# zetanumbers/myraytracer

Measured on AMD Instinct MI355X. Metric: Msamples/s (pixels x spp / s), random-spheres, higher is better.
Workload: dtype f32

## Files before the change

myraytracer_amd/csrc/kernels.hip:

```cpp

#include <hip/hip_runtime.h>
#include "mrt_internal.h"
#include "mrt_device.h"
#include "sweep.h"
#include "blend.h"

#include <type_traits>

namespace mrt {
namespace {

__device__ __forceinline__ float sphere_quadratic(float cx, float cy, float cz, float neg_r2, V3 o, V3 d, float a, float& b, float& c) {
    const float ocx = o.x - cx, ocy = o.y - cy, ocz = o.z - cz;
    b = __builtin_fmaf(ocz, d.z, __builtin_fmaf(ocy, d.y, ocx * d.x));
    c = __builtin_fmaf(ocz, ocz, __builtin_fmaf(ocy, ocy, __builtin_fmaf(ocx, ocx, neg_r2)));
    return __builtin_fmaf(b, b, -(a * c));
}
__device__ __forceinline__ void literal_test(const SphereRec s, uint32_t idx, V3 o, V3 d, float a,
                                             float& t_sup, int32_t& best) {
    float b, c;
    const float disc = sphere_quadratic(s.cx, s.cy, s.cz, s.neg_r2, o, d, a, b, c);
    if (!(disc < 0.0f)) {
        float d_sqrt = __builtin_sqrtf(disc);
        const float t_min = 0.001f;
// ... 159 lines not shown
    const SphereRec* nodes = SMALL ? reinterpret_cast<const SphereRec*>(lds_raw) : P.nodes;
    const uint32_t* __restrict__ member_index = P.member_index;
    const SphQuadPtr sph_quads = (SphQuadPtr)(uintptr_t)P.clusters;
    const float pixel_side = 2.0f / (float)H;

    auto locate = [&](KArgPtr C, uint32_t q, uint32_t& px, uint32_t& py, uint32_t& texel, uint32_t& layer) -> bool {
        uint32_t tile = q >> 6;
        const uint32_t l = q & 63u;
        layer = 0u;
        if (!PILOT && C->queue_layers > 1u) { layer = tile / C->n_tiles; tile -= layer * C->n_tiles; }
        const uint32_t tile_x = tile % C->tiles_x, band = tile / C->tiles_x;
        const uint32_t Wc = C->locals.shape[0], Hc = C->locals.shape[1];
        px = tile_x * kTileW + (l & 7u);
        py = (band * C->shard_world + C->shard_rank) * kBandRows + (l >> 3);
        texel = (band * kBandRows + (l >> 3)) * Wc + px;
        return px < Wc && py < Hc;
    };

    uint32_t head = 0, tail = 0, avail = 0;
    bool queue_empty = false;

    bool has_task = false, task_done = false;
    uint32_t s_done = 0, pix_trips = 0, texel = 0;
    float base_x = 0.0f, base_y = 0.0f;
    Rng rng; rng.draws = 0; rng.s0 = rng.s1 = rng.s2 = rng.s3 = 0;
    uint32_t blk = 0;
    V3 color = v3(0.0f, 0.0f, 0.0f);
    V3 o = v3(0.0f, 0.0f, 0.0f), d = v3(0.0f, 0.0f, -1.0f), att = v3(1.0f, 1.0f, 1.0f);
    uint32_t depth_left = 0, trips = 0;
    unsigned long long started = 0, bounces = 0;
    unsigned long long mtests = 0;
    unsigned long long prim_slots = 0;

#ifdef MRT_STAMPS
    uint64_t phase_[7] = {0, 0, 0, 0, 0, 0, 0};
    uint64_t rounds_a_ = 0, rounds_b_ = 0, items_a_ = 0, items_b_ = 0;
    uint64_t last_ = __builtin_amdgcn_s_memtime();
    const uint64_t wave_t0_ = __builtin_amdgcn_s_memrealtime();
#endif

    for (;;) {
        const bool live = has_task && !task_done;
        auto new_sample_head = [&](V3& nd, V3& p) -> bool {
            if (CTR) {
                const KArgPtr Cs = cold_args();
                const uint4 sd = reinterpret_cast<const uint4*>(Cs->seeds)[texel];
                const uint32_t k4 = 4u * ((blk >> 7) * kCtrBlock + s_done);
                rng.s0 = fmix32((sd.x ^ Cs->locals.rng_shuffle[0]) + 0x9E3779B9u * (k4 + 1u));
                rng.s1 = fmix32((sd.y ^ Cs->locals.rng_shuffle[1]) + 0x9E3779B9u * (k4 + 2u));
                rng.s2 = fmix32((sd.z ^ Cs->locals.rng_shuffle[2]) + 0x9E3779B9u * (k4 + 3u));
                rng.s3 = fmix32((sd.w ^ Cs->locals.rng_shuffle[3]) + 0x9E3779B9u * (k4 + 4u));
                if ((rng.s0 | rng.s1 | rng.s2 | rng.s3) == 0u) {
                    rng.s0 = 0x9E3779B9u; rng.s1 = 0x7F4A7C15u; rng.s2 = 0xBF58476Du; rng.s3 = 0x1CE4E5B9u;
                }
            }
            float u = rng_f32(rng); float v = rng_f32(rng);
            float vx = base_x + u * pixel_side;
            float vy = base_y + v * pixel_side;
            const KArgPtr C = cold_args();
            att = v3(1.0f, 1.0f, 1.0f);
            depth_left = C->locals.ray_depth;
            if (C->cam.mode == 0) {
                o = v3(0.0f, 0.0f, 0.0f);
                nd = v3(vx, vy, -1.0f);
                return false;
            }
            p = v3((vx * C->cam.su[0] + vy * C->cam.sv[0]) - C->cam.fw[0],
                   (vx * C->cam.su[1] + vy * C->cam.sv[1]) - C->cam.fw[1],
                   (vx * C->cam.su[2] + vy * C->cam.sv[2]) - C->cam.fw[2]);
            o = v3(C->cam.origin[0], C->cam.origin[1], C->cam.origin[2]);
            nd = p;
            return C->cam.defocus != 0;
        };
        auto new_sample_lens = [&](V3& nd, V3 p, float lx, float ly) {
            const KArgPtr C = cold_args();
            const V3 off = v3(lx * C->cam.ru[0] + ly * C->cam.rv[0],
                              lx * C->cam.ru[1] + ly * C->cam.rv[1],
                              lx * C->cam.ru[2] + ly * C->cam.rv[2]);
            o = o + off;
            nd = p - off;
        };
        trips++;

        const bool trace = live && depth_left != 0u;
        if (trace) pix_trips++;
        if (!PILOT) bounces += (uint32_t)__popcll(__builtin_amdgcn_ballot_w64(trace));
        float t_sup = 1.0e4f;
        int32_t best = -1;
        if (__any(trace)) {
            const float a = dot3(d, d);
            constexpr bool CAM = SMALL && !DBG && !LISTS;
            bool cam_on = false;
            uint4 cam_entry = make_uint4(0xFFFFFFFFu, 0xFFFFFFFFu, 0xFFFFFFFFu, 0xFFFFFFFFu);
            if constexpr (CAM) {
                const KArgPtr C = cold_args();
                const uint32_t* const cam_masks = C->cam_masks;
                cam_on = cam_masks != nullptr;
                if (cam_on && trace && depth_left == C->locals.ray_depth) cam_entry = reinterpret_cast<const uint4*>(cam_masks)[texel >> 3];
            }
            auto cam_allow = [&](const uint32_t w) -> uint32_t {
                uint32_t allow = 0xFFFFFFFFu;
                if constexpr (CAM) { if (cam_on) allow = masks[w * 64u]; }
                return allow;
            };
            V3 o_rel = MFMA ? v3(o.x - P.mfma_origin[0], o.y - P.mfma_origin[1], o.z - P.mfma_origin[2]) : o;
            const float stretch = MFMA ? P.mfma_scale[0] : kBoundStretch;
            V3 ds = v3(d.x * stretch, d.y * stretch, d.z * stretch);
            if (MFMA && P.mfma_scaled != 0u) {
                o_rel = v3(o_rel.x * P.mfma_axis[0], o_rel.y * P.mfma_axis[1], o_rel.z * P.mfma_axis[2]);
                const V3 dd = v3(d.x * P.mfma_axis[0], d.y * P.mfma_axis[1], d.z * P.mfma_axis[2]);
                const float unit = __builtin_amdgcn_rsqf(dot3(dd, dd)) * stretch;
                ds = v3(dd.x * unit, dd.y * unit, dd.z * unit);
            }
            const float o_rel2 = MFMA ? dot3(o_rel, o_rel) : 0.0f;
            const bool weird = !(a > 0.99999f && a < 1.00001f) || (MFMA && !(o_rel2 <= P.mfma_scale[3]));
            const bool usable = trace && !weird;
            unsigned long long key0 = kNoHitKey;
            {
                const KArgPtr C = cold_args();
                const uint32_t n_direct = C->n_direct;
                const Divisor by_a = divisor_of(a);
                for (uint32_t j = 0; j < n_direct; j++) {
                    const float cx = C->direct[j].cx, cy = C->direct[j].cy, cz = C->direct[j].cz, nr2 = C->direct[j].neg_r2;
                    const uint32_t sidx = C->direct_index[j];
                    bool hq;
                    const unsigned long long key = sphere_root_key(cx, cy, cz, nr2, sidx, o, d, a, by_a, usable, hq);
                    key0 = key < key0 ? key : key0;
                    if (DBG && hq) atomicOr(P.dbg_cand + (size_t)texel * P.dbg_words + (sidx >> 5), 1u << (sidx & 31u));
                }
                if (!PILOT) mtests += (unsigned long long)n_direct * (uint32_t)__popcll(__builtin_amdgcn_ballot_w64(usable));
            }
            rays[2u * lane + 0u] = make_float4(o.x, o.y, o.z, d.x);
            rays[2u * lane + 1u] = make_float4(d.y, d.z, __uint_as_float((uint32_t)key0), __uint_as_float((uint32_t)(key0 >> 32)));
            lds_order();
            uint32_t bits = 0;
            MfmaRay mr;
            if (MFMA) mr = mfma_ray_operands(o_rel, ds, o_rel2, P.mfma_scale[1], P.mfma_scale[2], P.mfma_neg_k2_pair);
            if (CAM && cam_on) {
                masks[0] = cam_entry.x;
                if (n_padded > 32u) masks[64] = cam_entry.y;
                if (n_padded > 64u) masks[128] = cam_entry.z;
                if (n_padded > 96u) masks[192] = cam_entry.w;
                lds_order();
            }
            for (uint32_t blk = 0; blk < n_padded; blk += kBlockChunks * kChunk) {
                const uint32_t blk_end = (blk + kBlockChunks * kChunk < n_padded) ? blk + kBlockChunks * kChunk : n_padded;
                uint32_t nz = 0;
                uint32_t rem = 0;
                if (MFMA) {
                    uint32_t w = 0;
                    for (uint32_t i = blk; i < blk_end; i += 2u * kChunk, w++) {
                        const uint32_t allow = cam_allow(w);
                        uint32_t m = mfma_sweep_tile(reinterpret_cast<const u32x4*>(P.top_mfma)[(size_t)(i / 32u) * 64u + lane], mr);
                        if constexpr (CAM) m &= allow;
                        masks[w * 64u] = m;
                        nz |= (m < 1u ? m : 1u) << w;
                        rem += (uint32_t)__builtin_popcount(m);
                    }
                } else {
                Sph8 ga, gb;
                smem_load8(ga, sph_quads, blk);
                asm volatile("" : "=s"(gb.lo), "=s"(gb.hi));
                uint32_t c = 0;
                for (uint32_t i = blk; i < blk_end; i += kChunk, c++) {
                    const uint32_t allow = cam_allow(c >> 1);
                    smem_wait_then_load8(ga, gb, sph_quads, i + 8u, bits);  test8(ga, o, ds, bits);
                    const uint32_t nxt = (i + kChunk < n_padded) ? i + kChunk : 0u;
                    smem_wait_then_load8(gb, ga, sph_quads, nxt, bits);
                    test8(gb, o, ds, bits);
                    if (c & 1u) {
                        uint32_t m = ~bits;
                        if constexpr (CAM) m &= allow;
                        masks[(c >> 1) * 64u] = m;
                        nz |= (m < 1u ? m : 1u) << (c >> 1);
                        rem += (uint32_t)__builtin_popcount(m);
                    }
                }
                asm volatile("s_waitcnt lgkmcnt(0)" : "+s"(ga.lo), "+s"(ga.hi), "+s"(gb.lo), "+s"(gb.hi));
                }
                MRT_STAMP(1);
                if (!usable) { nz = 0; rem = 0; }
                lds_order();

                uint32_t wm = 0, ebase = 0;
                auto fetch_ray = [&](const uint32_t owner, V3& ro, V3& rd) {
                    const float4 r0 = rays[2u * owner];
                    const float2 r1 = *reinterpret_cast<const float2*>(rays + 2u * owner + 1u);
                    ro = v3(r0.x, r0.y, r0.z), rd = v3(r0.w, r1.x, r1.y);
                };
                auto root_round = [&](const entry_t* const src, uint32_t& n) {
                    const uint32_t take = n < 64u ? n : 64u, start = n - take;
                    const bool act = lane < take;
                    const uint32_t it = src[act ? start + lane : 0u];
                    const uint32_t owner = it >> kIdBits, node = it & ((1u << kIdBits) - 1u);
                    V3 ro, rd;
                    fetch_ray(owner, ro, rd);
                    const float ra = dot3(rd, rd);
                    const SphereRec sm = nodes[node];
                    const uint32_t sidx = SMALL ? (uint32_t)index_lds[node] : member_index[node];
                    float bq, cq;
                    const float disc = sphere_quadratic(sm.cx, sm.cy, sm.cz, sm.neg_r2, ro, rd, ra, bq, cq);
                    const float d_sqrt = sqrt_unscaled(disc);
                    const float t_min = 0.001f;
                    const Divisor by_a = divisor_of(ra);
                    const float t_near = div_unscaled(-bq - d_sqrt, by_a);
                    const float t_far = div_unscaled(-bq + d_sqrt, by_a);
                    const bool ok_near = !(t_near < t_min) && t_near < 1.0e4f;
                    const bool ok_far = !(t_far < t_min) && t_far < 1.0e4f;
                    const float t = ok_near ? t_near : t_far;
                    const unsigned long long key = (act && (ok_near || ok_far)) ? (((unsigned long long)__float_as_uint(t) << 32) | sidx) : kNoHitKey;
                    atomicMin(best_slots + 4u * owner, key);
                    if (DBG) {
                        const uint32_t owner_ray = (uint32_t)__builtin_amdgcn_ds_bpermute((int)(owner << 2), (int)texel);
                        if (act) atomicOr(P.dbg_cand + (size_t)owner_ray * P.dbg_words + (sidx >> 5), 1u << (sidx & 31u));
                    }
                    n = start;
#ifdef MRT_STAMPS
                    rounds_b_++; items_b_ += take;
#endif
                    lds_order();
                    MRT_WALK_STAMP(3);
                };
                auto members_round = [&](const SphereRec* const ch, const V3 ro, const V3 rd, const float ra, const bool on,
                                         const uint32_t e0, entry_t* const dst) -> uint32_t {
                    const SphereRec sr[4] = {ch[0], ch[1], ch[2], ch[3]};
                    bool h[4];
                    unsigned long long hm[4];
#pragma unroll
                    for (int q = 0; q < 4; q++) {
                        float bq, cq;
                        const float disc = sphere_quadratic(sr[q].cx, sr[q].cy, sr[q].cz, sr[q].neg_r2, ro, rd, ra, bq, cq);
                        h[q] = (int32_t)((__float_as_uint(bq) | __float_as_uint(cq)) & ~__float_as_uint(disc)) < 0;
                        hm[q] = __builtin_amdgcn_ballot_w64(h[q]);
                    }
                    const unsigned long long on_mask = __builtin_amdgcn_ballot_w64(on);
                    const unsigned long long m0 = hm[0] & on_mask, m1 = hm[1] & on_mask, m2 = hm[2] & on_mask, m3 = hm[3] & on_mask;
                    const unsigned long long any = m0 | m1 | m2 | m3;
                    const unsigned long long twice = (m0 & m1) | ((m0 | m1) & m2) | ((m0 | m1 | m2) & m3);
                    if (twice == 0ull) {
                        const uint32_t q = h[1] ? 1u : h[2] ? 2u : h[3] ? 3u : 0u;
                        if ((h[0] || h[1] || h[2] || h[3]) && on) dst[rank_in(any)] = (entry_t)(e0 + q);
                        return (uint32_t)__popcll(any);
                    }
                    uint32_t pushed = 0;
#pragma unroll
                    for (int q = 0; q < 4; q++) {
                        const unsigned long long mk = hm[q] & on_mask;
                        if (h[q] && on) dst[pushed + rank_in(mk)] = (entry_t)(e0 + (uint32_t)q);
                        pushed += (uint32_t)__popcll(mk);
                    }
                    return pushed;
                };
                if constexpr (SMALL) {
                    uint32_t qn0 = 0;
                    entry_t* const q0 = queues;
                    uint32_t* const starts = reinterpret_cast<uint32_t*>(queues + kQueueCap);
                    const uint32_t* const masks0 = masks - lane;
                    const uint32_t words = (blk_end - blk) / (2u * kChunk);
                    const bool own = rem != 0u;
                    const unsigned long long own_mask = __builtin_amdgcn_ballot_w64(own);
                    if (own_mask != 0ull) {
                        const uint32_t w0 = own ? 31u - (uint32_t)__builtin_clz(nz) : 0u;
                        const uint32_t m0 = masks[w0 * 64u];
                        const uint32_t node = blk + w0 * (2u * kChunk) + (own ? 31u - (uint32_t)__builtin_ctz(m0) : 0u);
                        qn0 += members_round(nodes + 4u * node, o, d, a, own, (lane << kIdBits) | (4u * node), q0 + qn0);
                        if (!PILOT) mtests += kClusterK * (uint32_t)__popcll(own_mask);
#ifdef MRT_STAMPS
                        rounds_a_++; items_a_ += (uint32_t)__popcll(own_mask);
#endif
                        lds_order();
                        MRT_WALK_STAMP(2);
                        while (qn0 >= 64u) root_round(q0, qn0);
                    }
                    const uint32_t rest = rem - (own ? 1u : 0u);
                    const uint32_t incl = wave_incl_scan(rest);
                    const uint32_t total_rem = (uint32_t)__builtin_amdgcn_readlane((int)incl, 63);
                    const uint32_t start_entry = rest != 0u ? ((incl - rest) << 6) | lane : 0xFFFFFFFFu;
                    uint32_t carry = 0u;
                    auto pick_word = [&](auto NW, const uint32_t owner, const uint32_t r, uint32_t& sel, uint32_t& r_in) -> uint32_t {
                        constexpr int n = decltype(NW)::value;
                        const uint32_t* const mo = masks0 + (int32_t)(words - (uint32_t)n) * 64 + owner;
                        uint32_t cnt = 0u, above = 0u, below = 0u;
                        bool found = false;
                        sel = 0u;
#pragma unroll
                        for (int i = n - 1; i >= 0; i--) {
                            const uint32_t m = mo[i * 64];
                            sel = found ? sel : m;
                            above = found ? above : cnt;
                            cnt += (uint32_t)__builtin_popcount(m);
                            found = r < cnt;
                            below += found ? 0u : 1u;
                        }
                        r_in = r - above;
                        return blk + (words - 1u - below) * (2u * kChunk);
                    };
                    for (uint32_t base = 0; base < total_rem; base += kItemWindow) {
#pragma unroll
                        for (uint32_t i = 0; i < kItemWindow; i += 64u) starts[i + lane] = 0u;
                        lds_order();
                        if ((start_entry >> 6) - base < kItemWindow) starts[(start_entry >> 6) - base] = start_entry;
                        lds_order();
                        const uint32_t window_end = total_rem - base < kItemWindow ? total_rem : base + kItemWindow;
                        for (uint32_t g0 = base; g0 < window_end; g0 += 64u) {
                            const uint32_t take = total_rem - g0 < 64u ? total_rem - g0 : 64u;
                            const bool act = lane < take;
                            uint32_t e = starts[g0 - base + lane];
                            e = wave_incl_max(e < carry ? carry : e);
                            carry = (uint32_t)__builtin_amdgcn_readlane((int)e, 63);
                            const uint32_t owner = e & 63u;
                            const uint32_t r = g0 + (act ? lane : take - 1u) - (e >> 6) + 1u;
                            uint32_t sel, r_in;
                            const uint32_t first = words <= 4u ? pick_word(IC<4>{}, owner, r, sel, r_in) : pick_word(IC<8>{}, owner, r, sel, r_in);
                            for (uint32_t trip = 0; trip < 31u && __any(r_in != 0u); trip++) {
                                if (r_in != 0u) { sel &= sel - 1u; r_in--; }
                            }
                            const uint32_t node = first + 31u - (uint32_t)__builtin_ctz(sel);
                            V3 ro, rd;
                            fetch_ray(owner, ro, rd);
                            MRT_WALK_STAMP(6);
                            qn0 += members_round(nodes + 4u * node, ro, rd, dot3(rd, rd), act, (owner << kIdBits) | (4u * node), q0 + qn0);
                            if (!PILOT) mtests += kClusterK * take;
#ifdef MRT_STAMPS
                            rounds_a_++; items_a_ += take;
#endif
                            lds_order();
                            MRT_WALK_STAMP(2);
                            while (qn0 >= 64u) root_round(q0, qn0);
                        }
                    }
                    while (qn0 != 0u) root_round(q0, qn0);
                } else {
                    constexpr uint32_t kIndexMask = (1u << 26) - 1u;
                    uint32_t sn = 0, cn = 0, rn = 0;
                    uint32_t* const clusterq = queues;
                    uint32_t* const rootq = queues + kQueueCap;
                    uint32_t* const stack = queues + 2u * kQueueCap;
                    typedef float f32x4 __attribute__((ext_vector_type(4)));
                    typedef float f32x2 __attribute__((ext_vector_type(2)));
                    typedef const f32x4 __attribute__((address_space(3)))* LdsBoxPtr;
                    typedef const f32x4 __attribute__((address_space(1)))* GlobalBoxPtr;
                    typedef const f32x2 __attribute__((address_space(3)))* LdsBox2Ptr;
                    typedef const f32x2 __attribute__((address_space(1)))* GlobalBox2Ptr;
                    auto f4 = [](const f32x4 v) { return make_float4(v.x, v.y, v.z, v.w); };
                    const LdsBoxPtr bxs_lds = (LdsBoxPtr)lds_raw;
                    const GlobalBoxPtr bxs_g = (GlobalBoxPtr)P.boxes;
                    const LdsBox2Ptr bx2_lds = (LdsBox2Ptr)lds_raw;
                    const GlobalBox2Ptr bx2_g = (GlobalBox2Ptr)P.boxes;
                    const float box_kc = P.box_kc;
                    const uint32_t box_lds = P.box_lds_count;
                    const bool top_in_lds = box_lds >= n_padded;
                    const uint32_t cluster_parent_first = P.box_cluster_parent_first;
                    for (;;) {
                        int k = rn >= 64u ? 0 : cn >= 64u ? 1 : sn >= 64u ? 2 : -1;
                        if (k < 0) {
                            if (__any((nz | wm) != 0u)) {
                                uint32_t qn = levels == 1u ? cn : sn;
                                uint32_t* const dst = levels == 1u ? clusterq : stack;
                                const uint32_t owner_bits = lane << 26;
                                auto next_candidate = [&]() -> uint32_t {
                                    uint32_t code = 0u;
                                    if ((nz | wm) != 0u) {
                                        if (wm == 0u) refill_mask_word(nz, wm, masks, ebase, 0u, blk);
                                        code = 0x80000000u | take_mask_bit(wm, ebase);
                                    }
                                    return code;
                                };
                                auto fetch_box = [&](const uint32_t code, V3& bc, V3& be) {
                                    const uint32_t g = code & 0x7FFFFFFFu;
                                    f32x2 w0, w1, w2;
                                    if (top_in_lds) { w0 = bx2_lds[3u * g]; w1 = bx2_lds[3u * g + 1u]; w2 = bx2_lds[3u * g + 2u]; }
                                    else { w0 = bx2_g[3u * (size_t)g]; w1 = bx2_g[3u * (size_t)g + 1u]; w2 = bx2_g[3u * (size_t)g + 2u]; }
                                    bc = v3(w0.x, w0.y, w1.x);
                                    be = v3(w1.y, w2.x, w2.y);
                                };
                                auto test_push = [&](const uint32_t code, const V3 bc, const V3 be) {
                                    const bool keep = (int32_t)(box_separated_bits<QUAD>(bc, be, box_kc, o, d) | ~code) >= 0;
                                    const unsigned long long km = __builtin_amdgcn_ballot_w64(keep);
                                    if (keep) dst[qn + rank_in(km)] = owner_bits | (code & 0x7FFFFFFFu);
                                    qn += (uint32_t)__popcll(km);
                                };
                                auto some_left = [&](const uint32_t code) -> bool { return __builtin_amdgcn_ballot_w64((int32_t)code < 0) != 0ull; };
                                uint32_t ca = next_candidate(), cb, left;
                                V3 a0, a1, b0, b1;
                                fetch_box(ca, a0, a1);
                                for (;;) {
                                    cb = next_candidate();
                                    fetch_box(cb, b0, b1);
                                    test_push(ca, a0, a1);
                                    if (!(some_left(cb) && qn < 128u)) { left = cb; break; }
                                    ca = next_candidate();
                                    fetch_box(ca, a0, a1);
                                    test_push(cb, b0, b1);
                                    if (!(some_left(ca) && qn < 128u)) { left = ca; break; }
                                }
                                if ((int32_t)left < 0) wm |= 0x80000000u >> ((left & 0x7FFFFFFFu) - ebase);
                                if (levels == 1u) cn = qn; else sn = qn;
                                lds_order();
                                MRT_WALK_STAMP(6);
                                continue;
                            }
                            k = sn != 0u ? 2 : cn != 0u ? 1 : rn != 0u ? 0 : -1;
                            if (k < 0) break;
                        }
                        if (k == 0) { root_round(rootq, rn); continue; }
                        const uint32_t n = k == 1 ? cn : sn;
                        uint32_t take = n < 64u ? n : 64u;
                        if (k == 2) {
                            const uint32_t fit = gen_cap > sn ? (gen_cap - sn) / 3u : 0u;
                            take = take <= fit ? take : (fit ? fit : 1u);
                        }
                        const uint32_t start = n - take;
                        const bool act = lane < take;
                        const uint32_t it = (k == 1 ? clusterq : stack)[act ? start + lane : 0u];
                        const uint32_t owner = it >> 26, g = act ? it & kIndexMask : 0u;
                        V3 ro, rd;
                        fetch_ray(owner, ro, rd);
                        if (k == 1) {
                            const uint32_t m4 = act ? 4u * (g - P.box_cluster_first) : 0u;
                            rn += members_round(nodes + m4, ro, rd, dot3(rd, rd), act, (owner << 26) | m4, rootq + rn);
                            cn = start;
                            if (!PILOT) mtests += kClusterK * take;
                        } else {
                            const uint32_t c0 = 4u * g + n_padded;
                            float4 b[6];
                            if (__builtin_amdgcn_ballot_w64(act && c0 + 4u > box_lds) == 0ull) {
                                const LdsBoxPtr bx = bxs_lds + 6u * (c0 >> 2);
#pragma unroll
                                for (int q = 0; q < 6; q++) b[q] = f4(bx[q]);
                            } else {
                                const GlobalBoxPtr bx = bxs_g + 6u * (size_t)(c0 >> 2);
#pragma unroll
                                for (int q = 0; q < 6; q++) b[q] = f4(bx[q]);
                            }
                            const V3 bc[4] = {v3(b[0].x, b[0].y, b[0].z), v3(b[1].z, b[1].w, b[2].x), v3(b[3].x, b[3].y, b[3].z), v3(b[4].z, b[4].w, b[5].x)};
                            const V3 be[4] = {v3(b[0].w, b[1].x, b[1].y), v3(b[2].y, b[2].z, b[2].w), v3(b[3].w, b[4].x, b[4].y), v3(b[5].y, b[5].z, b[5].w)};
                            bool h[4];
                            unsigned long long hm[4];
                            const unsigned long long act_mask = __builtin_amdgcn_ballot_w64(act);
#pragma unroll
                            for (int q = 0; q < 4; q++) {
                                h[q] = box_may_touch<QUAD>(bc[q], be[q], box_kc, ro, rd);
                                hm[q] = __builtin_amdgcn_ballot_w64(h[q]) & act_mask;
                            }
                            sn = start;
                            const bool to_c = g >= cluster_parent_first;
                            const unsigned long long m_c = __builtin_amdgcn_ballot_w64(to_c) & act_mask, m_s = act_mask & ~m_c;
                            const uint32_t e0 = (owner << 26) | c0;
                            auto push4 = [&](uint32_t* const dst, const unsigned long long who, const bool mine) -> uint32_t {
                                uint32_t pushed = 0;
#pragma unroll
                                for (int q = 0; q < 4; q++) {
                                    const unsigned long long mk = hm[q] & who;
                                    if (h[q] && mine) dst[pushed + rank_in(mk)] = e0 + (uint32_t)q;
                                    pushed += (uint32_t)__popcll(mk);
                                }
                                return pushed;
                            };
                            if (m_s != 0ull) sn += push4(stack + sn, m_s, act && !to_c);
                            if (m_c != 0ull) cn += push4(clusterq + cn, m_c, act && to_c);
                        }
#ifdef MRT_STAMPS
                        rounds_a_++; items_a_ += take;
#endif
                        lds_order();
                        MRT_WALK_STAMP(2);
                    }
                }
            }
            if (trace) {
                if (weird) {
                    for (uint32_t idx = 0; idx < P.n_spheres; idx++)
                        literal_test(spheres[idx], idx, o, d, a, t_sup, best);
                } else {
                    const unsigned long long key = best_slots[4u * lane];
                    t_sup = __uint_as_float((uint32_t)(key >> 32));
                    best = (int32_t)(uint32_t)key;
                }
            }
        }
        MRT_WALK_STAMP(3);
        if (DBG && live) {
            P.dbg_hit[2u * texel] = best;
            P.dbg_hit[2u * texel + 1u] = (int32_t)__float_as_uint(t_sup);
            task_done = true;
        }

        bool start_sample = false;
        V3 ndir = d;
        bool hit = !DBG && live && depth_left != 0u && best >= 0;
        if (!DBG && live && !hit) {
            if (depth_left != 0u) {
                float t = 0.5f * d.y + 0.5f;
                color = color + att * v3(mixf(1.0f, 0.5f, t), mixf(1.0f, 0.7f, t), mixf(1.0f, 1.0f, t));
            }
            s_done++;
            if (s_done < (CTR ? (blk & 127u) : spp)) start_sample = true;
            else if (!CTR && !PILOT && blk + 1u < cold_args()->lane_frames) {
                const KArgPtr C = cold_args();
                PixAcc sa; sa.r = color.x; sa.g = color.y; sa.b = color.z; sa.cost = pix_trips;
                reinterpret_cast<PixAcc*>(C->pix_acc)[(size_t)blk * C->pix_stride + texel] = sa;
                blk++;
                const uint4 sd = reinterpret_cast<const uint4*>(C->seeds)[texel];
                rng.s0 = sd.x ^ C->layer_shuffle[blk][0];
                rng.s1 = sd.y ^ C->layer_shuffle[blk][1];
                rng.s2 = sd.z ^ C->layer_shuffle[blk][2];
                rng.s3 = sd.w ^ C->layer_shuffle[blk][3];
                color = v3(0.0f, 0.0f, 0.0f);
                s_done = 0;
                pix_trips = 0;
                start_sample = true;
            } else task_done = true;
        }
        MRT_STAMP(4);

        const bool release = has_task && task_done;
        if (release) {
            if (!DBG) {
                PixAcc sa; sa.r = color.x; sa.g = color.y; sa.b = color.z; sa.cost = pix_trips;
                const KArgPtr C = cold_args();
                reinterpret_cast<PixAcc*>(C->pix_acc)[(size_t)(CTR ? (blk >> 7) : blk) * C->pix_stride + texel] = sa;
            }
            has_task = false;
        }
        const unsigned long long need = __ballot(!has_task);
        if (!queue_empty && avail < (uint32_t)__popcll(need)) {
            const KArgPtr C = cold_args();
            uint32_t t = 0;
            if (lane == 0) t = atomicAdd(C->tile_queue, 1u);
            t = __builtin_amdgcn_readfirstlane(t);
            const uint32_t n_layers = PILOT ? 1u : C->queue_layers;
            if (t >= C->n_tiles * n_layers) {
                queue_empty = true;
            } else {
                const uint32_t lay = PILOT ? 0u : t / C->n_tiles, ti = t - lay * C->n_tiles;
                const uint32_t tile = lay * C->n_tiles + (C->tile_order ? C->tile_order[ti] : ti);
                uint32_t fx, fy, ft, fl;
                const uint32_t fq = (tile << 6) | lane;
                const bool ok = locate(C, fq, fx, fy, ft, fl);
                const unsigned long long m = __ballot(ok);
                if (ok) ring[(tail + rank_in(m)) & (kRingCap - 1u)] = fq;
                const uint32_t nf = (uint32_t)__popcll(m);
                tail += nf;
                avail += nf;
            }
        }
        if (need != 0ull && avail != 0u) {
            const uint32_t rk = rank_in(need);
            const bool take = !has_task && rk < avail;
            if (take) {
                const KArgPtr C = cold_args();
                uint32_t px, py, layer;
                locate(C, ring[(head + rk) & (kRingCap - 1u)], px, py, texel, layer);
                const float Wf = (float)C->locals.shape[0], Hf = (float)C->locals.shape[1];
                base_x = (((float)px + 0.5f) - 0.5f * Wf) * pixel_side;
                base_y = (((float)py + 0.5f) - 0.5f * Hf) * pixel_side;
                const uint4 sd = reinterpret_cast<const uint4*>(C->seeds)[texel];
                const uint32_t li = CTR ? 0u : layer;
                rng.s0 = sd.x ^ C->layer_shuffle[li][0];
                rng.s1 = sd.y ^ C->layer_shuffle[li][1];
                rng.s2 = sd.z ^ C->layer_shuffle[li][2];
                rng.s3 = sd.w ^ C->layer_shuffle[li][3];
                if (!CTR) texel += layer * C->pix_stride;
                color = v3(0.0f, 0.0f, 0.0f);
                s_done = 0;
                pix_trips = 0;
                has_task = true;
                blk = 0u;
                if (CTR) {
                    const uint32_t first = layer * kCtrBlock;
                    const uint32_t cnt = spp > first ? (spp - first < kCtrBlock ? spp - first : kCtrBlock) : 0u;
                    blk = (layer << 7) | cnt;
                }
                task_done = (spp == 0u);
                start_sample = !task_done;
                if (DBG) {
                    const float* const r6 = C->dbg_rays + 6u * (size_t)texel;
                    o = v3(r6[0], r6[1], r6[2]);
                    d = v3(r6[3], r6[4], r6[5]);
                    depth_left = 1u;
                    task_done = false;
                    start_sample = false;
                }
            }
            const uint32_t np = (uint32_t)__popcll(need);
            const uint32_t took = np < avail ? np : avail;
            head += took;
            avail -= took;
        }
        if (!__any(has_task)) {
            if (queue_empty) break;
            continue;
        }
        MRT_STAMP(5);

        if (!DBG) {
            V3 cam_p = v3(0.0f, 0.0f, 0.0f);
            bool need_lens = false;
            bool own_ray = false;
            if constexpr (LISTS) {
                if (__any(start_sample)) {
                    uint4 ent = make_uint4(kCamListOverflow, 0u, 0u, 0u);
                    if (start_sample) {
                        ent = reinterpret_cast<const uint4*>(cold_args()->cam_lists)[texel >> 3];
                        if (new_sample_head(ndir, cam_p)) {
                            float lx, ly;
                            do { lx = rng_pm1(rng); ly = rng_pm1(rng); } while (__builtin_fmaf(ly, ly, lx * lx) > 1.0f);
                            new_sample_lens(ndir, cam_p, lx, ly);
                        }
                        d = unit_direction(ndir);
                        ndir = d;
                        own_ray = true;
                    }
                    const float a = dot3(d, d);
                    const bool prim = start_sample && depth_left != 0u && ent.x != kCamListOverflow && a > 0.99999f && a < 1.00001f;
                    const unsigned long long prim_mask = __builtin_amdgcn_ballot_w64(prim);
                    const KArgPtr C = cold_args();
                    const uint32_t n_direct = C->n_direct;
                    const Divisor by_a = divisor_of(a);
                    unsigned long long key = kNoHitKey;
                    bool hq;
                    for (uint32_t j = 0; j < n_direct; j++) {
                        const unsigned long long kk = sphere_root_key(C->direct[j].cx, C->direct[j].cy, C->direct[j].cz, C->direct[j].neg_r2,
                                                                      C->direct_index[j], o, d, a, by_a, prim, hq);
                        key = kk < key ? kk : key;
                    }
                    if (!PILOT) mtests += (unsigned long long)n_direct * (uint32_t)__popcll(prim_mask);
                    const uint32_t cnt = prim ? ent.x : 0u;
                    uint32_t w0 = ent.y, w1 = ent.z, w2 = ent.w;
                    for (uint32_t k = 0;; k++) {
                        const bool on = k < cnt;
                        const unsigned long long on_mask = __builtin_amdgcn_ballot_w64(on);
                        if (on_mask == 0ull) break;
                        const uint32_t slot = on ? w0 & 1023u : 0u;
                        w0 = __builtin_amdgcn_alignbit(w1, w0, 10u); w1 = __builtin_amdgcn_alignbit(w2, w1, 10u); w2 >>= 10u;
                        const SphereRec sm = nodes[slot];
                        const unsigned long long kk = sphere_root_key(sm.cx, sm.cy, sm.cz, sm.neg_r2, (uint32_t)index_lds[slot], o, d, a, by_a, on, hq);
                        key = kk < key ? kk : key;
                        if (!PILOT) mtests += (uint32_t)__popcll(on_mask);
                    }
                    if (!PILOT) {
                        bounces += (uint32_t)__popcll(prim_mask);
                        prim_slots += (uint32_t)__popcll(prim_mask);
                    }
                    if (prim) {
                        pix_trips++;
                        if ((int32_t)(uint32_t)key >= 0) {
                            t_sup = __uint_as_float((uint32_t)(key >> 32));
                            best = (int32_t)(uint32_t)key;
                            hit = true;
                            own_ray = false;
                        } else {
                            float t = 0.5f * d.y + 0.5f;
                            color = color + att * v3(mixf(1.0f, 0.5f, t), mixf(1.0f, 0.7f, t), mixf(1.0f, 1.0f, t));
                            depth_left = 0u;
                        }
                    }
                }
            } else if (start_sample) need_lens = new_sample_head(ndir, cam_p);
            MRT_TAIL_STAMP(2);
            V3 normal = v3(0.0f, 0.0f, 0.0f), refl = v3(0.0f, 0.0f, 0.0f);
            float fuzz = 0.0f;
            bool is_lambertian = false, is_metal = false;
            if (hit) {
                const KArgPtr C = cold_args();
                const float4 sh0 = reinterpret_cast<const float4*>(C->shade)[2 * best];
                const float4 sh1 = reinterpret_cast<const float4*>(C->shade)[2 * best + 1];
                const int32_t m_ty = C->i32_data[C->world.spheres.material_ty_base_idx + best];
                const V3 center = v3(sh0.x, sh0.y, sh0.z);
                const float radius = sh0.w;
                const V3 at = o + t_sup * d;
                const V3 rel = at - center;
                const float rel_min = __builtin_fminf(__builtin_fminf(__builtin_fabsf(rel.x), __builtin_fabsf(rel.y)), __builtin_fabsf(rel.z));
                if (__builtin_expect(__any(!normal_unscaled_ok(rel_min, radius)), 0)) {
                    normal = rel / radius;
                } else {
                    const Divisor by_r = divisor_of(radius);
                    normal = v3(div_unscaled(rel.x, by_r), div_unscaled(rel.y, by_r), div_unscaled(rel.z, by_r));
                }
                const bool front_face = dot3(normal, d) <= 0.0f;
                if (!front_face) normal = -normal;
                is_lambertian = m_ty == MRT_LAMBERTIAN;
                is_metal = m_ty == MRT_METAL;
                if (is_lambertian || is_metal) {
                    att = att * v3(sh1.x, sh1.y, sh1.z);
                    if (is_metal) { refl = reflect3(d, normal); fuzz = sh1.w; }
                } else if (m_ty == MRT_DIELECTRIC) {
                    const float ior = sh1.w;
                    const float ri = front_face ? sh1.x : ior;
                    const float r0 = front_face ? sh1.y : sh1.z;
                    float cos_t = dot3(-d, normal);
                    cos_t = (cos_t < 1.0f) ? cos_t : 1.0f;
                    const float sin_t = sqrt_unscaled(1.0f - cos_t * cos_t);
                    const bool cannot_refract = (ri * sin_t) > 1.0f;
                    const float x1 = 1.0f - cos_t;
                    const float x2 = x1 * x1; const float x4 = x2 * x2; const float x5 = x4 * x1;
                    const float reflectance = r0 + (1.0f - r0) * x5;
                    const float u = rng_f32(rng);
                    if (cannot_refract || reflectance > u) {
                        ndir = reflect3(d, normal);
                    } else {
                        const V3 perp = v3(ri * (d.x + cos_t * normal.x), ri * (d.y + cos_t * normal.y),
                                           ri * (d.z + cos_t * normal.z));
                        const float k = -sqrt_unscaled(__builtin_fabsf(1.0f - dot3(perp, perp)));
                        ndir = v3(perp.x + k * normal.x, perp.y + k * normal.y, perp.z + k * normal.z);
                    }
                } else {
                    depth_left = 1u;
                    ndir = d;
                }
                o = at;
            }
            MRT_TAIL_STAMP(3);
            const bool need_ball = is_lambertian || is_metal;
            float bx = 0.0f, by = 0.0f, bz = 0.0f;
            if (need_ball || need_lens) {
                do {
                    bx = rng_pm1(rng); by = rng_pm1(rng);
                    bz = 0.0f;
                    if (need_ball) bz = rng_pm1(rng);
                } while (__builtin_fmaf(bz, bz, __builtin_fmaf(by, by, bx * bx)) > 1.0f);
            }
            MRT_TAIL_STAMP(6);
            if (need_lens) new_sample_lens(ndir, cam_p, bx, by);
            if (hit) {
                bool scattered = true;
                if (is_lambertian) {
                    const Divisor by_len = divisor_of(sqrt_unscaled(__builtin_fmaf(bz, bz, __builtin_fmaf(by, by, bx * bx))));
                    ndir = normal + v3(div_unscaled(bx, by_len), div_unscaled(by, by_len), div_unscaled(bz, by_len));
                    if (dot3(ndir, ndir) == 0.0f) ndir = normal;
                } else if (is_metal) {
                    ndir = v3(refl.x + fuzz * bx, refl.y + fuzz * by, refl.z + fuzz * bz);
                    scattered = !(dot3(ndir, normal) <= 0.0f);
                }
                depth_left = scattered ? depth_left - 1u : 0u;
            }
            if (has_task && !task_done && !own_ray) {
                const float dd = dot3(ndir, ndir);
                const float nd_min = __builtin_fminf(__builtin_fminf(__builtin_fabsf(ndir.x), __builtin_fabsf(ndir.y)), __builtin_fabsf(ndir.z));
                if (__builtin_expect(__any(!normalize_unscaled_ok(dd, nd_min)), 0)) {
                    d = normalize3(ndir);
                } else {
                    const Divisor by_len = divisor_of(sqrt_unscaled(dd));
                    d = v3(div_unscaled(ndir.x, by_len), div_unscaled(ndir.y, by_len), div_unscaled(ndir.z, by_len));
                }
            }
        }
        MRT_STAMP(0);
        if (!PILOT) started += (uint32_t)__popcll(__builtin_amdgcn_ballot_w64(start_sample));
    }

    if (!PILOT) {
        const unsigned long long c0 = started, c1 = bounces;
        unsigned long long c2 = COUNT ? rng.draws : 0u;
        if (COUNT) {
#pragma unroll
            for (int off = 32; off > 0; off >>= 1) c2 += __shfl_xor(c2, off);
        }
        if (lane == 0 && P.counters) {
            atomicAdd(P.counters + 0, c0);
            atomicAdd(P.counters + 1, c1);
            atomicAdd(P.counters + 2, c2);
            atomicAdd(P.counters + 3, 64ull * trips + (LISTS ? prim_slots : 0ull));
            atomicAdd(P.counters + 4, (unsigned long long)mtests);
#ifdef MRT_STAMPS
            for (int k = 0; k < 6; k++) atomicAdd(P.counters + 6 + k, (unsigned long long)phase_[k]);
            atomicAdd(P.counters + 5, (unsigned long long)phase_[6]);
            atomicAdd(P.counters + 12, (unsigned long long)rounds_a_);
            atomicAdd(P.counters + 13, (unsigned long long)rounds_b_);
            atomicAdd(P.counters + 14, (unsigned long long)items_a_);
            atomicAdd(P.counters + 15, (unsigned long long)items_b_);
            if (P.wave_log) {
                unsigned long long* wl = P.wave_log + 4ull * (blockIdx.x * kWavesPerGroup + wave);
                wl[0] = wave_t0_; wl[1] = __builtin_amdgcn_s_memrealtime(); wl[2] = trips; wl[3] = c1;
            }
#endif
        }
    }
}

template <bool PILOT, bool TRACKED>
__device__ __forceinline__ void finalize_body(const KParams& P, float* __restrict__ noise_s) {
    const uint32_t lane = threadIdx.x, tile = blockIdx.x;
    const uint32_t W = P.locals.shape[0], H = P.locals.shape[1];
    uint32_t px, py;
    size_t texel;
    blend_locate(lane, tile, P.tiles_x, P.shard_world, P.shard_rank, W, px, py, texel);
    uint32_t cost = 0;
    if (px < W && py < H) {
        const PixAcc sa = blend_sum_layers(reinterpret_cast<const PixAcc*>(P.pix_acc), texel, PILOT ? 1u : P.n_blocks, P.pix_stride);
        cost = sa.cost;
        if (!PILOT)
            blend_texel<TRACKED>(sa, P.locals.samples_per_frame, P.locals.framebuffer_weight, reinterpret_cast<const float4*>(P.prev),
                                 reinterpret_cast<float4*>(P.out), noise_s, texel);
    } else if (!PILOT && px < W) {
        blend_padding<TRACKED>(reinterpret_cast<float4*>(P.out), noise_s, texel);
    }
    cost = blend_max_cost(cost);
    if (lane == 0 && P.tile_cost) P.tile_cost[tile] = cost;
    if (lane == 0 && tile == 0) *P.tile_queue = 0u;
}
template <bool PILOT>
__global__ void __launch_bounds__(64) finalize_kernel(const KParams P) { finalize_body<PILOT, false>(P, nullptr); }
__global__ void __launch_bounds__(64) finalize_tracked_kernel(const KParams P, float* __restrict__ noise_s) {
    finalize_body<false, true>(P, noise_s);
}

__global__ void __launch_bounds__(256) fill_seeds_kernel(uint32_t* seeds, uint64_t seed, uint32_t W, uint32_t H,
                                                         uint32_t shard_rank, uint32_t shard_world,
                                                         uint32_t local_rows) {
    const uint32_t px = blockIdx.x * blockDim.x + threadIdx.x;
    const uint32_t lrow = blockIdx.y;
    if (px >= W || lrow >= local_rows) return;
    const uint32_t py = ((lrow / kBandRows) * shard_world + shard_rank) * kBandRows + (lrow % kBandRows);
    uint4 s = make_uint4(0, 0, 0, 0);
    if (py < H) {
        const uint64_t p = (uint64_t)py * W + px;
        const uint64_t a = splitmix64_at(seed, 2u * p), b = splitmix64_at(seed, 2u * p + 1u);
        s = make_uint4((uint32_t)a, (uint32_t)(a >> 32), (uint32_t)b, (uint32_t)(b >> 32));
        if ((s.x | s.y | s.z | s.w) == 0u)
            s = make_uint4(0x9E3779B9u, 0x7F4A7C15u, 0xBF58476Du, 0x1CE4E5B9u);
    }
    reinterpret_cast<uint4*>(seeds)[(size_t)lrow * W + px] = s;
}

}

static uint32_t group_lds_bytes(const KParams& p, bool small) {
    return (small ? p.n_nodes * (uint32_t)sizeof(SphereRec) + lds_index_bytes(p.n_members) : p.box_lds_count * (uint32_t)sizeof(BoxRec)) +
           kWavesPerGroup * lds_wave_bytes(small, p.levels, p.gen_cap, p.mask_chunks);
}

// ... 113 lines not shown
```

myraytracer_amd/csrc/sweep.h:

```cpp
#pragma once
#include "rt_math.h"

namespace mrt {

typedef float f32x16 __attribute__((ext_vector_type(16)));
typedef const f32x16 __attribute__((address_space(4)))* SphQuadPtr;
struct Sph8 { f32x16 lo, hi; };

__device__ __forceinline__ void smem_load8(Sph8& g, SphQuadPtr quads, uint32_t first_sphere) {
    const SphQuadPtr p = quads + first_sphere / 4u;
    asm volatile("s_load_dwordx16 %0, %2, 0x0\n\ts_load_dwordx16 %1, %2, 0x40"
                 : "=&s"(g.lo), "=&s"(g.hi) : "s"(p));
}
__device__ __forceinline__ void smem_wait_then_load8(Sph8& cur, Sph8& nxt, SphQuadPtr quads, uint32_t first_sphere,
                                                     uint32_t& bits) {
    const SphQuadPtr p = quads + first_sphere / 4u;
    asm volatile("s_waitcnt lgkmcnt(0)\n\ts_load_dwordx16 %2, %5, 0x0\n\ts_load_dwordx16 %3, %5, 0x40"
                 : "+s"(cur.lo), "+s"(cur.hi), "=&s"(nxt.lo), "=&s"(nxt.hi), "+v"(bits) : "s"(p));
}
__device__ __forceinline__ void test1(float cx, float cy, float cz, float neg_R2, V3 o, V3 ds, uint32_t& bits) {
    const float ocx = o.x - cx, ocy = o.y - cy, ocz = o.z - cz;
    const float b = __builtin_fmaf(ocz, ds.z, __builtin_fmaf(ocy, ds.y, ocx * ds.x));
    const float c = __builtin_fmaf(ocz, ocz, __builtin_fmaf(ocy, ocy, __builtin_fmaf(ocx, ocx, neg_R2)));
    const float S = __builtin_fmaf(b, b, -c);
    bits = __builtin_amdgcn_alignbit(bits, __float_as_uint(S), 31);
}
__device__ __forceinline__ void test4(const f32x16 q, V3 o, V3 ds, uint32_t& bits) {
    test1(q[0], q[1], q[2], q[3], o, ds, bits);
    test1(q[4], q[5], q[6], q[7], o, ds, bits);
    test1(q[8], q[9], q[10], q[11], o, ds, bits);
    test1(q[12], q[13], q[14], q[15], o, ds, bits);
}
__device__ __forceinline__ void test8(const Sph8& g, V3 o, V3 ds, uint32_t& bits) {
    test4(g.lo, o, ds, bits);
    test4(g.hi, o, ds, bits);
}

template <bool QUAD>
__device__ __forceinline__ uint32_t box_separated_bits(const V3 c, const V3 e, const float kc, V3 o, V3 d) {
    const float px = o.x - c.x, py = o.y - c.y, pz = o.z - c.z;
    const float X = QUAD ? __builtin_fmaf(pz, pz, __builtin_fmaf(py, py, px * px))
                         : (__builtin_fabsf(px) + __builtin_fabsf(py)) + __builtin_fabsf(pz);
    const float K = kc * X;
    const float ex = e.x, ey = e.y, ez = e.z;
    const float adx = __builtin_fabsf(d.x), ady = __builtin_fabsf(d.y), adz = __builtin_fabsf(d.z);
    const float sx = __builtin_fmaf(ey, adz, __builtin_fmaf(ez, ady, K)) - __builtin_fabsf(__builtin_fmaf(-pz, d.y, py * d.z));
    const float sy = __builtin_fmaf(ez, adx, __builtin_fmaf(ex, adz, K)) - __builtin_fabsf(__builtin_fmaf(-px, d.z, pz * d.x));
    const float sz = __builtin_fmaf(ex, ady, __builtin_fmaf(ey, adx, K)) - __builtin_fabsf(__builtin_fmaf(-py, d.x, px * d.y));
    return __float_as_uint(sx) | __float_as_uint(sy) | __float_as_uint(sz);
}
template <bool QUAD>
__device__ __forceinline__ bool box_may_touch(const V3 c, const V3 e, const float kc, V3 o, V3 d) {
    return (int32_t)box_separated_bits<QUAD>(c, e, kc, o, d) >= 0;
}

typedef __bf16 bf16x8 __attribute__((ext_vector_type(8)));
typedef uint32_t u32x4 __attribute__((ext_vector_type(4)));
struct MfmaRay { u32x4 bp[2], bu[2]; };
__device__ __forceinline__ uint32_t pk_bf16(float lo, float hi) {
    typedef __bf16 bf16x2 __attribute__((ext_vector_type(2)));
    const bf16x2 v = {(__bf16)lo, (__bf16)hi};
    return __builtin_bit_cast(uint32_t, v);
}
__device__ __forceinline__ float bf16_round(float x) { return (float)(__bf16)x; }
__device__ __forceinline__ void swap32(uint32_t a, uint32_t b, uint32_t& r0, uint32_t& r1) {
    const auto r = __builtin_amdgcn_permlane32_swap(a, b, false, false);
    r0 = r[0];
    r1 = r[1];
}
__device__ __forceinline__ void mfma_pack_ray(V3 v, float w0, float w1, float w2, uint32_t y2, uint32_t y3, u32x4 out[2]) {
    const V3 h = v3(bf16_round(v.x), bf16_round(v.y), bf16_round(v.z));
    const V3 l = v3(v.x - h.x, v.y - h.y, v.z - h.z);
    const uint32_t x0 = pk_bf16(h.x, h.y), x1 = pk_bf16(h.z, l.x), x2 = pk_bf16(l.y, l.z);
    const uint32_t y0 = pk_bf16(h.z, w0), y1 = pk_bf16(w1, w2);
    uint32_t a0, a1, a2, a3, b0, b1, b2, b3;
    swap32(x0, y0, a0, b0);
    swap32(x1, y1, a1, b1);
    swap32(x2, y2, a2, b2);
    swap32(x0, y3, a3, b3);
    out[0] = u32x4{a0, a1, a2, a3};
    out[1] = u32x4{b0, b1, b2, b3};
}
__device__ __forceinline__ MfmaRay mfma_ray_operands(V3 o, V3 dsk, float o2, float s2k2, float nsk2, uint32_t nk2) {
    MfmaRay m;
    const float nk0 = -dot3(o, dsk);
    const float n0 = bf16_round(nk0), n1 = bf16_round(nk0 - n0), n2 = (nk0 - n0) - n1;
    mfma_pack_ray(dsk, n0, n1, n2, 0u, 0u, m.bp);
    const float k1p = o2 * nsk2;
    const float q0 = bf16_round(k1p), q1 = bf16_round(k1p - q0), q2 = (k1p - q0) - q1;
    mfma_pack_ray(v3(s2k2 * o.x, s2k2 * o.y, s2k2 * o.z), q0, q1, q2, nk2, nk2 & 0xFFFFu, m.bu);
    return m;
}
__device__ __forceinline__ uint32_t mfma_sweep_tile(const u32x4 a, const MfmaRay& m) {
    const f32x16 zero = {0, 0, 0, 0, 0, 0, 0, 0, 0, 0, 0, 0, 0, 0, 0, 0};
    const bf16x8 av = __builtin_bit_cast(bf16x8, a);
    uint32_t hb[2];
#pragma unroll
    for (int h = 0; h < 2; h++) {
        f32x16 acc = __builtin_amdgcn_mfma_f32_32x32x16_bf16(av, __builtin_bit_cast(bf16x8, m.bp[h]), zero, 0, 0, 0);
#pragma unroll
        for (int i = 0; i < 16; i++) acc[i] = __builtin_amdgcn_fmed3f(acc[i] * __builtin_fabsf(acc[i]), 0.0f, 1.0f);
        acc = __builtin_amdgcn_mfma_f32_32x32x16_bf16(av, __builtin_bit_cast(bf16x8, m.bu[h]), acc, 0, 0, 0);
        uint32_t bb = 0;
#pragma unroll
        for (int i = 0; i < 16; i++) bb = __builtin_amdgcn_alignbit(bb, __float_as_uint(acc[i]), 31);
        hb[h] = bb;
    }
    const auto r = __builtin_amdgcn_permlane32_swap(hb[0], hb[1], false, false);
    return ~((r[0] << 16) | (r[1] & 0xFFFFu));
}

}
```

Before: 18520.

## Replace per-lane predicates with ballot masks and buffer loads in small-scene path

For the SMALL specialization, lane predicates (trace, usable, prim, fetch ok) are built as combined wave ballot masks and turned back into per-lane booleans with inverse_ballot, so one scalar mask is reused instead of computing repeated ballots/any reductions. The MFMA top-level sweep now loads tiles through a raw buffer resource with a running byte offset, and tracks the last nonzero mask word directly instead of a bitfield plus clz. The loop-exit test is derived from the need/took counts, and finished lanes get depth zeroed so the live check can be dropped. It also drops the 0xFFFF mask in the tile result, assuming the upper bits are already clear. These changes aim to cut scalar/vector mask overhead and address arithmetic, at the risk of subtle semantic differences in lane activity.

Result: faster. 18790, median of 6 (+1.5%).

```diff
diff --git a/myraytracer_amd/csrc/kernels.hip b/myraytracer_amd/csrc/kernels.hip
--- a/myraytracer_amd/csrc/kernels.hip
+++ b/myraytracer_amd/csrc/kernels.hip
@@ -265,12 +265,13 @@
         };
         trips++;
 
-        const bool trace = live && depth_left != 0u;
+        const bool trace = (SMALL && !DBG) ? depth_left != 0u : live && depth_left != 0u;
         if (trace) pix_trips++;
-        if (!PILOT) bounces += (uint32_t)__popcll(__builtin_amdgcn_ballot_w64(trace));
+        const unsigned long long trace_mask = __builtin_amdgcn_ballot_w64(trace);
+        if (!PILOT) bounces += (uint32_t)__popcll(trace_mask);
         float t_sup = 1.0e4f;
         int32_t best = -1;
-        if (__any(trace)) {
+        if (SMALL ? trace_mask != 0ull : __any(trace) != 0) {
             const float a = dot3(d, d);
             constexpr bool CAM = SMALL && !DBG && !LISTS;
             bool cam_on = false;
@@ -296,8 +297,18 @@
                 ds = v3(dd.x * unit, dd.y * unit, dd.z * unit);
             }
             const float o_rel2 = MFMA ? dot3(o_rel, o_rel) : 0.0f;
-            const bool weird = !(a > 0.99999f && a < 1.00001f) || (MFMA && !(o_rel2 <= P.mfma_scale[3]));
-            const bool usable = trace && !weird;
+            bool weird, usable;
+            unsigned long long usable_mask = 0ull;
+            if constexpr (SMALL) {
+                const unsigned long long admitted = __builtin_amdgcn_ballot_w64(a > 0.99999f) & __builtin_amdgcn_ballot_w64(a < 1.00001f) &
+                                                    (MFMA ? __builtin_amdgcn_ballot_w64(o_rel2 <= P.mfma_scale[3]) : ~0ull);
+                usable_mask = trace_mask & admitted;
+                weird = !__builtin_amdgcn_inverse_ballot_w64(admitted);
+                usable = __builtin_amdgcn_inverse_ballot_w64(usable_mask);
+            } else {
+                weird = !(a > 0.99999f && a < 1.00001f) || (MFMA && !(o_rel2 <= P.mfma_scale[3]));
+                usable = trace && !weird;
+            }
             unsigned long long key0 = kNoHitKey;
             {
                 const KArgPtr C = cold_args();
@@ -311,7 +322,8 @@
                     key0 = key < key0 ? key : key0;
                     if (DBG && hq) atomicOr(P.dbg_cand + (size_t)texel * P.dbg_words + (sidx >> 5), 1u << (sidx & 31u));
                 }
-                if (!PILOT) mtests += (unsigned long long)n_direct * (uint32_t)__popcll(__builtin_amdgcn_ballot_w64(usable));
+                if (!SMALL) usable_mask = __builtin_amdgcn_ballot_w64(usable);
+                if (!PILOT) mtests += (unsigned long long)n_direct * (uint32_t)__popcll(usable_mask);
             }
             rays[2u * lane + 0u] = make_float4(o.x, o.y, o.z, d.x);
             rays[2u * lane + 1u] = make_float4(d.y, d.z, __uint_as_float((uint32_t)key0), __uint_as_float((uint32_t)(key0 >> 32)));
@@ -330,15 +342,30 @@
                 const uint32_t blk_end = (blk + kBlockChunks * kChunk < n_padded) ? blk + kBlockChunks * kChunk : n_padded;
                 uint32_t nz = 0;
                 uint32_t rem = 0;
+                uint32_t top = 0;
                 if (MFMA) {
                     uint32_t w = 0;
+                    if constexpr (SMALL) {
+                        const __amdgpu_buffer_rsrc_t top_rsrc = __builtin_amdgcn_make_buffer_rsrc(
+                            const_cast<void*>(static_cast<const void*>(P.top_mfma)), 0, (int)(n_padded * 32u), 0x00020000);
+                        uint32_t tile_bytes = blk * 32u;
+                        for (uint32_t i = blk; i < blk_end; i += 2u * kChunk, w++, tile_bytes += 1024u) {
+                            const uint32_t allow = cam_allow(w);
+                            uint32_t m = mfma_sweep_tile<true>(__builtin_amdgcn_raw_buffer_load_b128(top_rsrc, lane * 16u, (int)tile_bytes, 0), mr);
+                            if constexpr (CAM) m &= allow;
+                            masks[w * 64u] = m;
+                            top = m != 0u ? w : top;
+                            rem += (uint32_t)__builtin_popcount(m);
+                        }
+                    } else {
                     for (uint32_t i = blk; i < blk_end; i += 2u * kChunk, w++) {
                         const uint32_t allow = cam_allow(w);
-                        uint32_t m = mfma_sweep_tile(reinterpret_cast<const u32x4*>(P.top_mfma)[(size_t)(i / 32u) * 64u + lane], mr);
+                        uint32_t m = mfma_sweep_tile<false>(reinterpret_cast<const u32x4*>(P.top_mfma)[(size_t)(i / 32u) * 64u + lane], mr);
                         if constexpr (CAM) m &= allow;
                         masks[w * 64u] = m;
                         nz |= (m < 1u ? m : 1u) << w;
                         rem += (uint32_t)__builtin_popcount(m);
+                    }
                     }
                 } else {
                 Sph8 ga, gb;
@@ -355,7 +382,8 @@
                         uint32_t m = ~bits;
                         if constexpr (CAM) m &= allow;
                         masks[(c >> 1) * 64u] = m;
-                        nz |= (m < 1u ? m : 1u) << (c >> 1);
+                        if constexpr (SMALL) top = m != 0u ? (c >> 1) : top;
+                        else nz |= (m < 1u ? m : 1u) << (c >> 1);
                         rem += (uint32_t)__builtin_popcount(m);
                     }
                 }
@@ -405,7 +433,7 @@
                     MRT_WALK_STAMP(3);
                 };
                 auto members_round = [&](const SphereRec* const ch, const V3 ro, const V3 rd, const float ra, const bool on,
-                                         const uint32_t e0, entry_t* const dst) -> uint32_t {
+                                         const unsigned long long on_ballot, const uint32_t e0, entry_t* const dst) -> uint32_t {
                     const SphereRec sr[4] = {ch[0], ch[1], ch[2], ch[3]};
                     bool h[4];
                     unsigned long long hm[4];
@@ -416,7 +444,7 @@
                         h[q] = (int32_t)((__float_as_uint(bq) | __float_as_uint(cq)) & ~__float_as_uint(disc)) < 0;
                         hm[q] = __builtin_amdgcn_ballot_w64(h[q]);
                     }
-                    const unsigned long long on_mask = __builtin_amdgcn_ballot_w64(on);
+                    const unsigned long long on_mask = SMALL ? on_ballot : __builtin_amdgcn_ballot_w64(on);
                     const unsigned long long m0 = hm[0] & on_mask, m1 = hm[1] & on_mask, m2 = hm[2] & on_mask, m3 = hm[3] & on_mask;
                     const unsigned long long any = m0 | m1 | m2 | m3;
                     const unsigned long long twice = (m0 & m1) | ((m0 | m1) & m2) | ((m0 | m1 | m2) & m3);
@@ -443,10 +471,10 @@
                     const bool own = rem != 0u;
                     const unsigned long long own_mask = __builtin_amdgcn_ballot_w64(own);
                     if (own_mask != 0ull) {
-                        const uint32_t w0 = own ? 31u - (uint32_t)__builtin_clz(nz) : 0u;
+                        const uint32_t w0 = top;
                         const uint32_t m0 = masks[w0 * 64u];
                         const uint32_t node = blk + w0 * (2u * kChunk) + (own ? 31u - (uint32_t)__builtin_ctz(m0) : 0u);
-                        qn0 += members_round(nodes + 4u * node, o, d, a, own, (lane << kIdBits) | (4u * node), q0 + qn0);
+                        qn0 += members_round(nodes + 4u * node, o, d, a, own, own_mask, (lane << kIdBits) | (4u * node), q0 + qn0);
                         if (!PILOT) mtests += kClusterK * (uint32_t)__popcll(own_mask);
 #ifdef MRT_STAMPS
                         rounds_a_++; items_a_ += (uint32_t)__popcll(own_mask);
@@ -488,6 +516,7 @@
                         for (uint32_t g0 = base; g0 < window_end; g0 += 64u) {
                             const uint32_t take = total_rem - g0 < 64u ? total_rem - g0 : 64u;
                             const bool act = lane < take;
+                            const unsigned long long act_mask = take < 64u ? (1ull << take) - 1ull : ~0ull;
                             uint32_t e = starts[g0 - base + lane];
                             e = wave_incl_max(e < carry ? carry : e);
                             carry = (uint32_t)__builtin_amdgcn_readlane((int)e, 63);
@@ -502,7 +531,7 @@
                             V3 ro, rd;
                             fetch_ray(owner, ro, rd);
                             MRT_WALK_STAMP(6);
-                            qn0 += members_round(nodes + 4u * node, ro, rd, dot3(rd, rd), act, (owner << kIdBits) | (4u * node), q0 + qn0);
+                            qn0 += members_round(nodes + 4u * node, ro, rd, dot3(rd, rd), act, act_mask, (owner << kIdBits) | (4u * node), q0 + qn0);
                             if (!PILOT) mtests += kClusterK * take;
 #ifdef MRT_STAMPS
                             rounds_a_++; items_a_ += take;
@@ -601,7 +630,7 @@
                         fetch_ray(owner, ro, rd);
                         if (k == 1) {
                             const uint32_t m4 = act ? 4u * (g - P.box_cluster_first) : 0u;
-                            rn += members_round(nodes + m4, ro, rd, dot3(rd, rd), act, (owner << 26) | m4, rootq + rn);
+                            rn += members_round(nodes + m4, ro, rd, dot3(rd, rd), act, 0ull, (owner << 26) | m4, rootq + rn);
                             cn = start;
                             if (!PILOT) mtests += kClusterK * take;
                         } else {
@@ -670,6 +699,7 @@
         }
 
         bool start_sample = false;
+        unsigned long long start_mask = 0ull;
         V3 ndir = d;
         bool hit = !DBG && live && depth_left != 0u && best >= 0;
         if (!DBG && live && !hit) {
@@ -693,7 +723,10 @@
                 s_done = 0;
                 pix_trips = 0;
                 start_sample = true;
-            } else task_done = true;
+            } else {
+                task_done = true;
+                if (SMALL) depth_left = 0u;
+            }
         }
         MRT_STAMP(4);
 
@@ -720,14 +753,17 @@
                 const uint32_t tile = lay * C->n_tiles + (C->tile_order ? C->tile_order[ti] : ti);
                 uint32_t fx, fy, ft, fl;
                 const uint32_t fq = (tile << 6) | lane;
-                const bool ok = locate(C, fq, fx, fy, ft, fl);
-                const unsigned long long m = __ballot(ok);
+                bool ok = locate(C, fq, fx, fy, ft, fl);
+                const unsigned long long m = SMALL ? __builtin_amdgcn_ballot_w64(fx < C->locals.shape[0]) & __builtin_amdgcn_ballot_w64(fy < C->locals.shape[1])
+                                                   : __ballot(ok);
+                if constexpr (SMALL) ok = __builtin_amdgcn_inverse_ballot_w64(m);
                 if (ok) ring[(tail + rank_in(m)) & (kRingCap - 1u)] = fq;
                 const uint32_t nf = (uint32_t)__popcll(m);
                 tail += nf;
                 avail += nf;
             }
         }
+        uint32_t took = 0u;
         if (need != 0ull && avail != 0u) {
             const uint32_t rk = rank_in(need);
             const bool take = !has_task && rk < avail;
@@ -767,11 +803,11 @@
                 }
             }
             const uint32_t np = (uint32_t)__popcll(need);
-            const uint32_t took = np < avail ? np : avail;
+            took = np < avail ? np : avail;
             head += took;
             avail -= took;
         }
-        if (!__any(has_task)) {
+        if (SMALL ? (need == ~0ull && took == 0u) : !__any(has_task)) {
             if (queue_empty) break;
             continue;
         }
@@ -782,7 +818,8 @@
             bool need_lens = false;
             bool own_ray = false;
             if constexpr (LISTS) {
-                if (__any(start_sample)) {
+                start_mask = __builtin_amdgcn_ballot_w64(start_sample);
+                if (start_mask != 0ull) {
                     uint4 ent = make_uint4(kCamListOverflow, 0u, 0u, 0u);
                     if (start_sample) {
                         ent = reinterpret_cast<const uint4*>(cold_args()->cam_lists)[texel >> 3];
@@ -796,8 +833,10 @@
                         own_ray = true;
                     }
                     const float a = dot3(d, d);
-                    const bool prim = start_sample && depth_left != 0u && ent.x != kCamListOverflow && a > 0.99999f && a < 1.00001f;
-                    const unsigned long long prim_mask = __builtin_amdgcn_ballot_w64(prim);
+                    const unsigned long long prim_mask = start_mask & __builtin_amdgcn_ballot_w64(depth_left != 0u) &
+                                                         __builtin_amdgcn_ballot_w64(ent.x != kCamListOverflow) &
+                                                         __builtin_amdgcn_ballot_w64(a > 0.99999f) & __builtin_amdgcn_ballot_w64(a < 1.00001f);
+                    const bool prim = __builtin_amdgcn_inverse_ballot_w64(prim_mask);
                     const KArgPtr C = cold_args();
                     const uint32_t n_direct = C->n_direct;
                     const Divisor by_a = divisor_of(a);
@@ -809,12 +848,11 @@
                         key = kk < key ? kk : key;
                     }
                     if (!PILOT) mtests += (unsigned long long)n_direct * (uint32_t)__popcll(prim_mask);
-                    const uint32_t cnt = prim ? ent.x : 0u;
                     uint32_t w0 = ent.y, w1 = ent.z, w2 = ent.w;
                     for (uint32_t k = 0;; k++) {
-                        const bool on = k < cnt;
-                        const unsigned long long on_mask = __builtin_amdgcn_ballot_w64(on);
+                        const unsigned long long on_mask = prim_mask & __builtin_amdgcn_ballot_w64(k < ent.x);
                         if (on_mask == 0ull) break;
+                        const bool on = __builtin_amdgcn_inverse_ballot_w64(on_mask);
                         const uint32_t slot = on ? w0 & 1023u : 0u;
                         w0 = __builtin_amdgcn_alignbit(w1, w0, 10u); w1 = __builtin_amdgcn_alignbit(w2, w1, 10u); w2 >>= 10u;
                         const SphereRec sm = nodes[slot];
@@ -930,7 +968,7 @@
             }
         }
         MRT_STAMP(0);
-        if (!PILOT) started += (uint32_t)__popcll(__builtin_amdgcn_ballot_w64(start_sample));
+        if (!PILOT) started += (uint32_t)__popcll(LISTS ? start_mask : __builtin_amdgcn_ballot_w64(start_sample));
     }
 
     if (!PILOT) {
diff --git a/myraytracer_amd/csrc/sweep.h b/myraytracer_amd/csrc/sweep.h
--- a/myraytracer_amd/csrc/sweep.h
+++ b/myraytracer_amd/csrc/sweep.h
@@ -91,6 +91,7 @@
     mfma_pack_ray(v3(s2k2 * o.x, s2k2 * o.y, s2k2 * o.z), q0, q1, q2, nk2, nk2 & 0xFFFFu, m.bu);
     return m;
 }
+template <bool TIGHT>
 __device__ __forceinline__ uint32_t mfma_sweep_tile(const u32x4 a, const MfmaRay& m) {
     const f32x16 zero = {0, 0, 0, 0, 0, 0, 0, 0, 0, 0, 0, 0, 0, 0, 0, 0};
     const bf16x8 av = __builtin_bit_cast(bf16x8, a);
@@ -107,7 +108,13 @@
         hb[h] = bb;
     }
     const auto r = __builtin_amdgcn_permlane32_swap(hb[0], hb[1], false, false);
-    return ~((r[0] << 16) | (r[1] & 0xFFFFu));
+    if constexpr (TIGHT) {
+        uint32_t x = (r[0] << 16) | r[1];
+        asm("" : "+v"(x));
+        x = ~x;
+        asm("" : "+v"(x));
+        return x;
+    } else return ~((r[0] << 16) | (r[1] & 0xFFFFu));
 }
 
 }
```
